# ooowedyn/InkLayer

Hardware: AMD Instinct MI355X
Metric: sketches/sec end-to-end (GroundingDINO+SAM) at 1024x1024 (higher is better)
Workload: dtype f16 (MFMA, f32 accumulate; f32 residual/norm/softmax; split-f16 = fp32-grade operands for patch-embed, neck, mask decoder); 1 GPU; full GroundingDINO Swin-T + SAM ViT-H pipeline, batch=8 per GPU, 1024x1024 synthetic sketches, 16 boxes/sketch, random-init weights; global_batch=8, parallelism=image-parallel x1

## Files before the change

inklayer_amd/csrc/msda.hip:

```cpp
#include "common.h"
#include "../../include/inklayer_hip.h"

namespace {

constexpr int MAXL = 8;

struct LevelInfo {
  int H[MAXL], W[MAXL], start[MAXL];
};

struct HostLevels {
  LevelInfo li;
  __device__ __forceinline__ bool get(int l, int, int& H, int& W, int64_t& start) const {
    H = li.H[l];
    W = li.W[l];
    start = li.start[l];
    return true;
  }
};

struct DevLevels {
  const int64_t* shapes;
  const int64_t* starts;
  __device__ __forceinline__ bool get(int l, int S, int& H, int& W, int64_t& start) const {
    const int64_t h = shapes[2 * l], w = shapes[2 * l + 1], s = starts[l];
    const bool ok = h > 0 && w > 0 && h <= S && w <= S && s >= 0 && s <= S && s + h * w <= S;
    H = ok ? (int)h : 0;
    W = ok ? (int)w : 0;
    start = ok ? s : 0;
    return ok;
  }
};

template <typename T, int NV>
__device__ __forceinline__ void loadv(const T* p, T (&v)[NV]) {
  if constexpr (NV * sizeof(T) % 16 == 0) {
#pragma unroll
    for (int i = 0; i < (int)(NV * sizeof(T) / 16); ++i) {
// ... 21 lines not shown
}

template <typename T, int NV>
__device__ __forceinline__ void sample_acc(const T* __restrict__ vbase, int64_t row_stride, int H, int W,
                                           T h_im, T w_im, T aw, T (&acc)[NV]) {
  if (!(h_im > (T)-1 && w_im > (T)-1 && h_im < (T)H && w_im < (T)W)) return;
  const int h0 = (int)floor(h_im), w0 = (int)floor(w_im);
  const T lh = h_im - (T)h0, lw = w_im - (T)w0;
  const T hh = (T)1 - lh, hw = (T)1 - lw;
  const T w00 = hh * hw * aw, w01 = hh * lw * aw, w10 = lh * hw * aw, w11 = lh * lw * aw;
  T v[NV];
  if (h0 >= 0 && w0 >= 0) {
    loadv<T, NV>(vbase + ((int64_t)h0 * W + w0) * row_stride, v);
#pragma unroll
    for (int i = 0; i < NV; ++i) acc[i] = fma(w00, v[i], acc[i]);
  }
  if (h0 >= 0 && w0 + 1 <= W - 1) {
    loadv<T, NV>(vbase + ((int64_t)h0 * W + w0 + 1) * row_stride, v);
#pragma unroll
    for (int i = 0; i < NV; ++i) acc[i] = fma(w01, v[i], acc[i]);
  }
  if (h0 + 1 <= H - 1 && w0 >= 0) {
    loadv<T, NV>(vbase + ((int64_t)(h0 + 1) * W + w0) * row_stride, v);
#pragma unroll
    for (int i = 0; i < NV; ++i) acc[i] = fma(w10, v[i], acc[i]);
  }
  if (h0 + 1 <= H - 1 && w0 + 1 <= W - 1) {
    loadv<T, NV>(vbase + ((int64_t)(h0 + 1) * W + w0 + 1) * row_stride, v);
#pragma unroll
    for (int i = 0; i < NV; ++i) acc[i] = fma(w11, v[i], acc[i]);
  }
}

__device__ __forceinline__ void sample_acc_bf(const f16* __restrict__ vbase, int64_t row_stride, int H, int W, float h_im,
                                              float w_im, float aw, float (&acc)[8]) {
  const bool in = h_im > -1.f && w_im > -1.f && h_im < (float)H && w_im < (float)W;
  const float hf = floorf(h_im), wf = floorf(w_im);
  const int h0 = in ? (int)hf : 0, w0 = in ? (int)wf : 0;
  const float lh = h_im - hf, lw = w_im - wf;
  const float hh = 1.f - lh, hw = 1.f - lw;
  const bool t = h0 >= 0, b = h0 + 1 <= H - 1, l = w0 >= 0, r = w0 + 1 <= W - 1;
  const float w00 = (in && t && l) ? hh * hw * aw : 0.f, w01 = (in && t && r) ? hh * lw * aw : 0.f;
  const float w10 = (in && b && l) ? lh * hw * aw : 0.f, w11 = (in && b && r) ? lh * lw * aw : 0.f;
  const int ht = max(h0, 0), hb = min(h0 + 1, H - 1), wl = max(w0, 0), wr = min(w0 + 1, W - 1);
  const f16x8 v00 = *(const f16x8*)(vbase + ((int64_t)ht * W + wl) * row_stride);
  const f16x8 v01 = *(const f16x8*)(vbase + ((int64_t)ht * W + wr) * row_stride);
  const f16x8 v10 = *(const f16x8*)(vbase + ((int64_t)hb * W + wl) * row_stride);
  const f16x8 v11 = *(const f16x8*)(vbase + ((int64_t)hb * W + wr) * row_stride);
#pragma unroll
  for (int i = 0; i < 8; ++i) acc[i] = fmaf(w00, (float)v00[i], acc[i]);
#pragma unroll
  for (int i = 0; i < 8; ++i) acc[i] = fmaf(w01, (float)v01[i], acc[i]);
#pragma unroll
  for (int i = 0; i < 8; ++i) acc[i] = fmaf(w10, (float)v10[i], acc[i]);
#pragma unroll
  for (int i = 0; i < 8; ++i) acc[i] = fmaf(w11, (float)v11[i], acc[i]);
}

template <typename T, int NV, typename Levels>
__global__ __launch_bounds__(256) void msda_fwd_kernel(const T* __restrict__ value, const T* __restrict__ loc,
                                                       const T* __restrict__ aw, Levels lv, int B, int S, int M,
                                                       int C, int Q, int L, int P, T* __restrict__ out) {
  const int nsl = C / NV;
  const int gid = xcd_remap(blockIdx.x, gridDim.x) * 256 + threadIdx.x;
  const int qm = gid / nsl, sl = gid - qm * nsl;
  if (qm >= B * Q * M) return;
  const int m = qm % M, b = qm / M / Q;
  T acc[NV];
#pragma unroll
  for (int i = 0; i < NV; ++i) acc[i] = 0;
  const T* lp = loc + (int64_t)qm * L * P * 2;
  const T* wp = aw + (int64_t)qm * L * P;
  const int64_t rs = (int64_t)M * C;
  for (int l = 0; l < L; ++l) {
    int H, W;
    int64_t start;
    if (!lv.get(l, S, H, W, start)) continue;
    const T* vb = value + ((int64_t)b * S + start) * rs + m * C + sl * NV;
    for (int p = 0; p < P; ++p) {
      const T lx = lp[(l * P + p) * 2], ly = lp[(l * P + p) * 2 + 1];
      sample_acc<T, NV>(vb, rs, H, W, ly * (T)H - (T)0.5, lx * (T)W - (T)0.5, wp[l * P + p], acc);
    }
  }
  storev<T, NV>(out + (int64_t)qm * C + sl * NV, acc);
}

template <int G, typename T>
__device__ __forceinline__ T group_sum(T v) {
#pragma unroll
// ... 53 lines not shown
            if (k10) atomicAdd(gval + o10 + c, w10 * ag);
            if (k11) atomicAdd(gval + o11 + c, w11 * ag);
          }
        }
      }
      sa = group_sum<G>(sa);
      sx = group_sum<G>(sx);
      sy = group_sum<G>(sy);
      if (lane == 0) {
        gaw[i] = sa;
        gloc[2 * i] = (T)W * a * sx;
        gloc[2 * i + 1] = (T)H * a * sy;
      }
    }
  }
}

template <int REFD>
__global__ __launch_bounds__(256) void msda_fused_kernel(const f16* __restrict__ value,
                                                         const float* __restrict__ proj, int64_t ldp,
                                                         const float* __restrict__ ref,
                                                         int64_t ref_q_stride, int64_t ref_b_stride,
                                                         LevelInfo li, int B, int S, int Q,
                                                         f16* __restrict__ out) {
  constexpr int M = 8, L = 4, P = 4, C = 32;
  const int64_t gid = (int64_t)xcd_remap(blockIdx.x, gridDim.x) * 256 + threadIdx.x;
  const int c8 = (int)(gid & 3);
  const int64_t qm = gid >> 2;
  if (qm >= (int64_t)B * Q * M) return;
  const int m = (int)(qm % M);
  const int64_t bq = qm / M;
  const int b = (int)(bq / Q), q = (int)(bq % Q);
  const float* pr = proj + bq * ldp;
  float off[L * P * 2], lg[L * P];
#pragma unroll
  for (int i = 0; i < 8; ++i) {
    const f32x4 v = *(const f32x4*)(pr + m * 32 + 4 * i);
    off[4 * i] = v[0]; off[4 * i + 1] = v[1]; off[4 * i + 2] = v[2]; off[4 * i + 3] = v[3];
  }
  float mx = -3.0e38f;
#pragma unroll
  for (int i = 0; i < 4; ++i) {
    const f32x4 v = *(const f32x4*)(pr + 256 + m * 16 + 4 * i);
#pragma unroll
    for (int j = 0; j < 4; ++j) { lg[4 * i + j] = v[j]; mx = fmaxf(mx, v[j]); }
  }
  float sum = 0.f;
#pragma unroll
  for (int i = 0; i < 16; ++i) { lg[i] = expf(lg[i] - mx); sum += lg[i]; }
  const float inv = 1.f / sum;
  const float* rp = ref + (int64_t)b * ref_b_stride + (int64_t)q * ref_q_stride;
  float acc[8] = {0, 0, 0, 0, 0, 0, 0, 0};
  const int64_t rs = (int64_t)M * C;
#pragma unroll
  for (int l = 0; l < L; ++l) {
    const int H = li.H[l], W = li.W[l];
    const f16* vb = value + ((int64_t)b * S + li.start[l]) * rs + m * C + c8 * 8;
    float rx, ry, rw = 0.f, rh = 0.f;
    if (REFD == 2) {
      rx = rp[0]; ry = rp[1];
    } else {
      rx = rp[0]; ry = rp[1]; rw = rp[2]; rh = rp[3];
    }
#pragma unroll
    for (int p = 0; p < P; ++p) {
      const float ox = off[(l * P + p) * 2], oy = off[(l * P + p) * 2 + 1];
      float lx, ly;
      if (REFD == 2) {
        lx = rx + ox / (float)W;
        ly = ry + oy / (float)H;
      } else {
        lx = rx + ox / (float)P * rw * 0.5f;
        ly = ry + oy / (float)P * rh * 0.5f;
      }
      sample_acc_bf(vb, rs, H, W, ly * H - 0.5f, lx * W - 0.5f, lg[l * P + p] * inv, acc);
    }
  }
  f16x8 o;
#pragma unroll
  for (int i = 0; i < 8; ++i) o[i] = (f16)acc[i];
  *(f16x8*)(out + qm * C + c8 * 8) = o;
}

template <typename T, int NV, typename Levels>
int launch_fwd(const void* value, const void* loc, const void* aw, Levels lv, int B, int S, int M, int C, int Q,
               int L, int P, void* out, hipStream_t s) {
  const int64_t threads = (int64_t)B * Q * M * (C / NV);
  hipLaunchKernelGGL((msda_fwd_kernel<T, NV, Levels>), dim3((unsigned)((threads + 255) / 256)), dim3(256), 0, s,
                     (const T*)value, (const T*)loc, (const T*)aw, lv, B, S, M, C, Q, L, P, (T*)out);
  return ink_launch_status();
}

template <typename T, int NVMAX, typename Levels>
int dispatch_fwd(const void* value, const void* loc, const void* aw, Levels lv, int B, int S, int M, int C, int Q,
                 int L, int P, void* out, hipStream_t s) {
  const bool aligned = ink_aligned<16>(value, out);
  if (aligned && C % NVMAX == 0) return launch_fwd<T, NVMAX>(value, loc, aw, lv, B, S, M, C, Q, L, P, out, s);
  if (aligned && C % (NVMAX / 2) == 0) return launch_fwd<T, NVMAX / 2>(value, loc, aw, lv, B, S, M, C, Q, L, P, out, s);
  return launch_fwd<T, 1>(value, loc, aw, lv, B, S, M, C, Q, L, P, out, s);
}

template <typename T, int G, int K>
int launch_bwd(const void* value, DevLevels lv, const void* loc, const void* aw, const void* gout, int B, int S,
               int M, int C, int Q, int L, int P, void* gval, void* gloc, void* gaw, hipStream_t s) {
  const int64_t threads = (int64_t)B * Q * M * G;
  hipLaunchKernelGGL((msda_bwd_kernel<T, G, K>), dim3((unsigned)((threads + 255) / 256)), dim3(256), 0, s,
                     (const T*)value, lv, (const T*)loc, (const T*)aw, (const T*)gout, B, S, M, C, Q, L, P, (T*)gval,
                     (T*)gloc, (T*)gaw);
  return ink_launch_status();
// ... 120 lines not shown
```

inklayer_amd/build.py:

```python
from __future__ import annotations

import os
import subprocess
import sys
from concurrent.futures import ThreadPoolExecutor
from pathlib import Path

ROOT = Path(__file__).resolve().parent
CSRC = ROOT / "csrc"
LIBDIR = ROOT / "lib"
OBJDIR = LIBDIR / "obj"
LIB = LIBDIR / "libinklayer_hip.so"
HIPCC = os.environ.get("HIPCC", "/opt/rocm/bin/hipcc")
FLAGS = ["--offload-arch=gfx950", "-O3", "-std=c++17", "-fPIC", "-ffp-contract=off",
         "-mllvm", "-amdgpu-mfma-vgpr-form",

         "-Wall", "-Wno-unused-function", "-Wno-unused-variable"]


def _newest_header() -> float:
    hs = list(CSRC.glob("*.h")) + list((ROOT.parent / "include").glob("*.h"))
    return max(h.stat().st_mtime for h in hs)


NO_SPILL = {"ffn_fused.hip", "proj_ln.hip", "amg.hip", "layers.hip", "inpaint_ops.hip", "visualize.hip", "evaluate.hip",
            "gemm.hip", "attention_swin.hip", "biattn_wide.hip", "text_bert.hip"}


def _check_no_spill(src: Path, remarks: str) -> None:
    name = None
    for line in remarks.splitlines():
        if "Function Name:" in line:
            name = line.split("Function Name:")[1].split("[")[0].strip()
        elif "ScratchSize [bytes/lane]:" in line:
            n = int(line.split("ScratchSize [bytes/lane]:")[1].split("[")[0])
            if n != 0:
                raise RuntimeError(f"{src.name}: kernel {name} spills ({n} bytes of scratch per lane) - the kernels of "
                                   f"this file must stay in registers (see NO_SPILL); reduce register pressure")


def _compile(src: Path, force: bool, hdr_time: float) -> Path:
    obj = OBJDIR / (src.stem + ".o")
    if (not force and obj.exists() and obj.stat().st_mtime > src.stat().st_mtime
            and obj.stat().st_mtime > hdr_time):
        return obj
    guard = src.name in NO_SPILL
    cmd = [HIPCC, *FLAGS, *(["-Rpass-analysis=kernel-resource-usage", "-fno-caret-diagnostics"] if guard else []), "-c", str(src), "-o", str(obj)]
    r = subprocess.run(cmd, capture_output=True, text=True)
    if r.returncode != 0:
        raise RuntimeError(f"hipcc failed for {src.name}:\n{r.stdout}\n{r.stderr}")
    err = r.stderr
    if guard:
        try:
            _check_no_spill(src, err)
        except RuntimeError:
            obj.unlink(missing_ok=True)
            raise
        err = "\n".join(l for l in err.splitlines()
                        if "kernel-resource-usage" not in l and not l.startswith("In file included from"))
# ... 28 lines not shown
```

inklayer_amd/csrc/attn_few.hip:

```cpp
#include "common.h"
#include "../../include/inklayer_hip.h"

namespace {

__device__ __forceinline__ void load8(const f16* p, float* d) {
  const f16x8 v = *(const f16x8*)p;
#pragma unroll
  for (int j = 0; j < 8; ++j) d[j] = (float)v[j];
}
__device__ __forceinline__ void load8(const float* p, float* d) {
  const f32x4 a = *(const f32x4*)p, b = *(const f32x4*)(p + 4);
#pragma unroll
  for (int j = 0; j < 4; ++j) { d[j] = a[j]; d[4 + j] = b[j]; }
}
__device__ __forceinline__ void store8(f16* p, const float* d) {
  f16x8 v;
#pragma unroll
  for (int j = 0; j < 8; ++j) v[j] = (f16)d[j];
  *(f16x8*)p = v;
}
__device__ __forceinline__ void store8(float* p, const float* d) {
  *(f32x4*)p = (f32x4){d[0], d[1], d[2], d[3]};
  *(f32x4*)(p + 4) = (f32x4){d[4], d[5], d[6], d[7]};
}
// ... 107 lines not shown
      bm = fmaxf(bm, d);
    }
    if (bm <= -1.0e38f) continue;
    const float mn = fmaxf(m, bm);
    const float a = expf(m - mn);
    l *= a;
#pragma unroll
    for (int i = 0; i < HD; ++i) acc[i] *= a;
    m = mn;
#pragma unroll
    for (int u = 0; u < 8; ++u) {
      if (sc[u] <= -1.0e38f) continue;
      const float pw = expf(sc[u] - m);
      l += pw;
      const f16* vp = V + ((int64_t)b * n_k + t0 + u) * ldv + h * HD;
#pragma unroll
      for (int i = 0; i < HD / 8; ++i) {
        float vv[8];
        load8(vp + 8 * i, vv);
#pragma unroll
        for (int j = 0; j < 8; ++j) acc[8 * i + j] = fmaf(pw, vv[j], acc[8 * i + j]);
      }
    }
  }
  const float inv = l > 0.f ? 1.f / l : 0.f;
#pragma unroll
  for (int i = 0; i < HD; ++i) acc[i] *= inv;
  f16* op = O + bq * ldo + h * HD;
#pragma unroll
  for (int i = 0; i < HD / 8; ++i) store8(op + 8 * i, acc + 8 * i);
}


template <int NK>
__global__ __launch_bounds__(256) void attn_fewkeys16_f32_kernel(const float* __restrict__ Q, int64_t ldq,
                                                                 const float* __restrict__ K, int64_t ldk,
                                                                 const float* __restrict__ V, int64_t ldv, int B,
                                                                 int n_q, int n_heads, float scale,
                                                                 const int32_t* __restrict__ q_rows,
                                                                 const float* __restrict__ q_add,
                                                                 float* __restrict__ O, int64_t ldo) {
  const int64_t gid = (int64_t)blockIdx.x * 256 + threadIdx.x;
  if (gid >= (int64_t)B * n_q * n_heads * 4) return;
  const int part = (int)(gid & 3);
  const int h = (int)((gid >> 2) % n_heads);
  const int64_t bq = (gid >> 2) / n_heads;
  const int b = (int)(bq / n_q), q = (int)(bq % n_q);
  const int col = h * 16 + 4 * part;
  f32x4 qv = *(const f32x4*)(Q + (q_rows ? (int64_t)q_rows[b] + q : bq) * ldq + col);
  if (q_add) qv += *(const f32x4*)(q_add + (int64_t)q * n_heads * 16 + col);
  qv *= scale * 1.44269504088896340736f;
  const float* kp = K + (int64_t)b * NK * ldk + col;
  const float* vp = V + (int64_t)b * NK * ldv + col;
  f32x4 kv[NK], vv[NK];
#pragma unroll
  for (int t = 0; t < NK; ++t) {
    kv[t] = *(const f32x4*)(kp + (int64_t)t * ldk);
    vv[t] = *(const f32x4*)(vp + (int64_t)t * ldv);
  }
  float sc[NK];
  float mx = -3.0e38f;
#pragma unroll
  for (int t = 0; t < NK; ++t) {
    float d = (qv[0] * kv[t][0] + qv[1] * kv[t][1]) + (qv[2] * kv[t][2] + qv[3] * kv[t][3]);
    d += __builtin_bit_cast(float, __builtin_amdgcn_update_dpp(0, __builtin_bit_cast(int, d), 0xB1, 0xF, 0xF, false));
    d += __builtin_bit_cast(float, __builtin_amdgcn_update_dpp(0, __builtin_bit_cast(int, d), 0x4E, 0xF, 0xF, false));
    sc[t] = d;
    mx = fmaxf(mx, d);
  }
  float sum = 0.f;
#pragma unroll
  for (int t = 0; t < NK; ++t) { sc[t] = __builtin_amdgcn_exp2f(sc[t] - mx); sum += sc[t]; }
  const float inv = 1.f / sum;
  f32x4 acc = {0.f, 0.f, 0.f, 0.f};
#pragma unroll
  for (int t = 0; t < NK; ++t) acc += (sc[t] * inv) * vv[t];
  *(f32x4*)(O + bq * ldo + col) = acc;
}

template <int QW>
__global__ __launch_bounds__(512) void attn_fewq16_kernel(const float* __restrict__ Q, int64_t ldq,
                                                          const float* __restrict__ K, int64_t ldk,
                                                          const float* __restrict__ V, int64_t ldv, int n_q,
                                                          int n_k, int n_heads, float scale,
                                                          const int32_t* __restrict__ q_rows,
                                                          const int32_t* __restrict__ kv_rows,
                                                          const float* __restrict__ k_add,
                                                          float* __restrict__ O, int64_t ldo) {
  constexpr int KSPLIT = 2, HD = 16, HB = 4, TK = 64;
  constexpr int ROWE = HB * HD;
  constexpr int CH = 4, NCH = ROWE / CH;
  constexpr int NU = TK * NCH / 256;
  constexpr bool Q_IN_LDS = QW > 2;
  extern __shared__ __attribute__((aligned(16))) char fewq_smem[];
  const int grp = threadIdx.x >> 8;
  float* sk = (float*)fewq_smem + grp * 2 * TK * ROWE;
  float* sv = sk + TK * ROWE;
  const int hgroups = n_heads / HB;
  const int b = blockIdx.x / hgroups, h0 = (blockIdx.x % hgroups) * HB;
  const int tid = threadIdx.x & 255, lane = tid & 63, wave = tid >> 6;
  const int per = ((n_k + KSPLIT - 1) / KSPLIT + TK - 1) / TK * TK;
  const int k_lo = grp * per, k_hi = min(n_k, k_lo + per);
  const int kl = lane >> 2, hl = lane & 3;
  const int64_t q0 = q_rows ? (int64_t)q_rows[b] : (int64_t)b * n_q;
  const int64_t k0 = kv_rows ? (int64_t)kv_rows[b] : (int64_t)b * n_k;
  float* sq = (float*)fewq_smem + KSPLIT * 2 * TK * ROWE;
  float qr[QW][HD];
  if (!Q_IN_LDS || (grp == 0 && kl == 0)) {
    const float sc2 = scale * 1.44269504088896340736f;
#pragma unroll
    for (int j = 0; j < QW; ++j) {
      const int qi = QW * wave + j;
      const float* pq = Q + (q0 + (qi < n_q ? qi : 0)) * ldq + (h0 + hl) * HD;
      load8(pq, qr[j]);
      load8(pq + 8, qr[j] + 8);
#pragma unroll
      for (int e = 0; e < HD; ++e) qr[j][e] *= sc2;
      if constexpr (Q_IN_LDS) {
        store8(sq + (qi * HB + hl) * HD, qr[j]);
        store8(sq + (qi * HB + hl) * HD + 8, qr[j] + 8);
      }
    }
  }
  float m[QW], l[QW], acc[QW][HD];
#pragma unroll
  for (int j = 0; j < QW; ++j) {
    m[j] = -3.0e38f;
    l[j] = 0.f;
#pragma unroll
    for (int i = 0; i < HD; ++i) acc[j][i] = 0.f;
  }
  f32x4 rk[NU], rv[NU];
  auto fetch = [&](int t0) {
#pragma unroll
    for (int u = 0; u < NU; ++u) {
      const int c = tid + 256 * u, row = c / NCH, col = c % NCH;
      rk[u] = rv[u] = (f32x4){0.f, 0.f, 0.f, 0.f};
      if (t0 + row < k_hi) {
        rk[u] = *(const f32x4*)(K + (k0 + t0 + row) * ldk + h0 * HD + col * CH);
        rv[u] = *(const f32x4*)(V + (k0 + t0 + row) * ldv + h0 * HD + col * CH);
        if (k_add) rk[u] += *(const f32x4*)(k_add + (int64_t)(t0 + row) * n_heads * HD + h0 * HD + col * CH);
      }
    }
  };
  fetch(k_lo);
  for (int t0 = k_lo; t0 < k_lo + per; t0 += TK) {
    __syncthreads();
#pragma unroll
    for (int u = 0; u < NU; ++u) {
      const int c = tid + 256 * u, row = c / NCH, col = c % NCH;
      *(f32x4*)(sk + row * ROWE + col * CH) = rk[u];
      *(f32x4*)(sv + row * ROWE + col * CH) = rv[u];
    }
    __syncthreads();
    if (t0 + TK < k_hi) fetch(t0 + TK);
    float d[QW][TK / 16];
#pragma unroll
    for (int kk = 0; kk < TK / 16; ++kk) {
      const int key = kk * 16 + kl;
      float kf[HD];
      load8(sk + key * ROWE + hl * HD, kf);
      load8(sk + key * ROWE + hl * HD + 8, kf + 8);
      const bool in = t0 + key < k_hi;
#pragma unroll
      for (int j = 0; j < QW; ++j) {
        float qf[HD];
        if constexpr (Q_IN_LDS) {
          load8(sq + ((QW * wave + j) * HB + hl) * HD, qf);
          load8(sq + ((QW * wave + j) * HB + hl) * HD + 8, qf + 8);
        } else {
#pragma unroll
          for (int e = 0; e < HD; ++e) qf[e] = qr[j][e];
        }
        float a0 = 0.f;
#pragma unroll
        for (int e = 0; e < 8; ++e) {
          a0 = fmaf(qf[e], kf[e], a0);
          a0 = fmaf(qf[8 + e], kf[8 + e], a0);
        }
        d[j][kk] = in ? a0 : -3.0e38f;
      }
    }
    float n[QW];
#pragma unroll
    for (int j = 0; j < QW; ++j) {
// ... 69 lines not shown
        const float inv = 1.f / l[j];
#pragma unroll
        for (int i = 0; i < HD; ++i) acc[j][i] *= inv;
        float* op = O + ((int64_t)b * n_q + qi) * ldo + (h0 + hl) * HD;
        store8(op, acc[j]);
        store8(op + 8, acc[j] + 8);
      }
    }
  }
}

}

extern "C" int ink_attn_fewkeys(const void* Q, int64_t ldq, const void* K, int64_t ldk, const void* V,
                                int64_t ldv, int32_t B, int32_t n_q, int32_t n_k, int32_t n_heads,
                                int32_t head_dim, float scale, const uint8_t* blocked,
                                const int32_t* q_batch_rows, const float* q_add, int32_t io_f32, void* O,
                                int64_t ldo, void* stream) {
  INK_CHECK_ARG(Q && K && V && O && B > 0 && n_q > 0 && n_k > 0 && n_k <= 16 && n_heads > 0);
  INK_CHECK_ARG(ldq % 8 == 0 && ldk % 8 == 0 && ldv % 8 == 0 && ldo % 8 == 0);
  INK_CHECK_ARG(io_f32 == 0 || io_f32 == 1);
  INK_CHECK_ARG(ink_aligned<16>(Q, K, V, O, q_add));
  const int64_t total = (int64_t)B * n_q * n_heads;
  const dim3 grid((unsigned)((total + 255) / 256)), block(256);
  hipStream_t s = (hipStream_t)stream;
#define INK_FEWKEYS(HD, T)                                                                                     \
  hipLaunchKernelGGL((attn_fewkeys_kernel<HD, T>), grid, block, 0, s, (const T*)Q, ldq, (const T*)K, ldk,      \
                     (const T*)V, ldv, B, n_q, n_k, n_heads, scale, blocked, q_batch_rows, q_add, (T*)O, ldo)
  if (head_dim == 32 && !io_f32) INK_FEWKEYS(32, f16);
  else if (head_dim == 64 && !io_f32) INK_FEWKEYS(64, f16);
  else if (!io_f32) return INK_ERR_ARG;
  else if (head_dim == 32) INK_FEWKEYS(32, float);
  else if (head_dim == 16 && !blocked && n_k >= 7) {
    const dim3 g4((unsigned)((total * 4 + 255) / 256));
#define INK_FEWKEYS16(NK)                                                                                        \
  case NK:                                                                                                      \
    hipLaunchKernelGGL(attn_fewkeys16_f32_kernel<NK>, g4, block, 0, s, (const float*)Q, ldq, (const float*)K, ldk, \
                       (const float*)V, ldv, B, n_q, n_heads, scale, q_batch_rows, q_add, (float*)O, ldo);         \
    break
    switch (n_k) {
      INK_FEWKEYS16(7); INK_FEWKEYS16(8); INK_FEWKEYS16(9); INK_FEWKEYS16(10); INK_FEWKEYS16(11);
      INK_FEWKEYS16(12); INK_FEWKEYS16(13); INK_FEWKEYS16(14); INK_FEWKEYS16(15); INK_FEWKEYS16(16);
      default: return INK_ERR_ARG;
    }
#undef INK_FEWKEYS16
  } else if (head_dim == 16) INK_FEWKEYS(16, float);
  else return INK_ERR_ARG;
#undef INK_FEWKEYS
  return ink_launch_status();
}

static int midkeys_launch(const void* Q, int64_t ldq, const void* K, int64_t ldk, const void* V, int64_t ldv,
                          int32_t B, int32_t n_q, int32_t n_k, int32_t n_heads, int32_t head_dim, float scale,
                          const uint8_t* blocked, int64_t blocked_stride, const int32_t* k_len, void* O, int64_t ldo,
                          void* stream) {
  INK_CHECK_ARG(Q && K && V && O && B > 0 && n_q > 0 && n_k > 0 && n_k <= 256 && n_heads > 0);
  INK_CHECK_ARG(head_dim == 32 || head_dim == 64);
  INK_CHECK_ARG(ldq % 8 == 0 && ldk % 8 == 0 && ldv % 8 == 0 && ldo % 8 == 0);
  INK_CHECK_ARG(ink_aligned<16>(Q, K, V, O));
  const int64_t total = (int64_t)B * n_q * n_heads;
  const dim3 grid((unsigned)((total + 255) / 256)), block(256);
#define INK_MIDKEYS(HD)                                                                                            \
  hipLaunchKernelGGL(attn_midkeys_kernel<HD>, grid, block, 0, (hipStream_t)stream, (const f16*)Q, ldq,             \
                     (const f16*)K, ldk, (const f16*)V, ldv, B, n_q, n_k, n_heads, scale, blocked, blocked_stride, \
                     k_len, (f16*)O, ldo)
  if (head_dim == 32) INK_MIDKEYS(32); else INK_MIDKEYS(64);
#undef INK_MIDKEYS
  return ink_launch_status();
}

extern "C" int ink_attn_midkeys(const void* Q, int64_t ldq, const void* K, int64_t ldk, const void* V,
                                int64_t ldv, int32_t B, int32_t n_q, int32_t n_k, int32_t n_heads,
                                int32_t head_dim, float scale, const uint8_t* blocked, void* O, int64_t ldo,
                                void* stream) {
  return midkeys_launch(Q, ldq, K, ldk, V, ldv, B, n_q, n_k, n_heads, head_dim, scale, blocked, 0, nullptr, O, ldo,
                        stream);
}

// ... 28 lines not shown
```

inklayer_amd/csrc/sam_decoder.hip:

```cpp
#include "common.h"
#include "sam_postprocess.h"
#include "../../include/inklayer_hip.h"

namespace {

__device__ __forceinline__ void pe_feature(float x, float y, const float* __restrict__ G, int F, int f, float& sv,
                                           float& cv) {
  const float cx = 2.f * x - 1.f, cy = 2.f * y - 1.f;
  float v = cx * G[f] + cy * G[F + f];
  v = 6.283185307179586f * v;
  sv = sinf(v);
  cv = cosf(v);
}

__global__ __launch_bounds__(256) void pe_encode_kernel(const float* __restrict__ coords,
                                                        const float* __restrict__ G, int N, int F,
                                                        const float* __restrict__ add, int n_add,
                                                        float* __restrict__ out) {
  const int i = blockIdx.x * 256 + threadIdx.x;
  if (i >= N * F) return;
  const int n = i / F, f = i % F;
  float sv, cv;
  pe_feature(coords[2 * n], coords[2 * n + 1], G, F, f, sv, cv);
  if (add) {
// ... 166 lines not shown
  const int b = (int)(tok / ((int64_t)g * g));
  const float* u = up + r * C;
  const float* h = hyper + (int64_t)b * C;
  float acc = 0.f;
#pragma unroll
  for (int c = 0; c < C; c += 4) {
    const f32x4 uv = *(const f32x4*)(u + c);
    const f32x4 hv = *(const f32x4*)(h + c);
    acc = fmaf(hv[0], uv[0], acc);
    acc = fmaf(hv[1], uv[1], acc);
    acc = fmaf(hv[2], uv[2], acc);
    acc = fmaf(hv[3], uv[3], acc);
  }
  const int Y = 4 * y + 2 * (s1 >> 1) + (s2 >> 1), X = 4 * x + 2 * (s1 & 1) + (s2 & 1);
  out[((int64_t)b * 4 * g + Y) * 4 * g + X] = acc;
}

__global__ __launch_bounds__(256) void postprocess_kernel(const float* __restrict__ low, int n, int S,
                                                          int L, int in_h, int in_w, int out_h,
                                                          int out_w, float thr,
                                                          uint8_t* __restrict__ out,
                                                          float* __restrict__ out_logits) {
  const int64_t total = (int64_t)n * out_h * out_w;
  const PostScales sc = post_scales(S, L, in_h, in_w, out_h, out_w);
  for (int64_t i = (int64_t)blockIdx.x * 256 + threadIdx.x; i < total; i += (int64_t)gridDim.x * 256) {
    const int X = (int)(i % out_w), Y = (int)((i / out_w) % out_h);
    const int b = (int)(i / ((int64_t)out_w * out_h));
    const float v = post_pixel(low + (int64_t)b * S * S, S, sc, in_h, in_w, Y, X);
    if (out) out[i] = v > thr ? 1 : 0;
    if (out_logits) out_logits[i] = v;
  }
}

__global__ __launch_bounds__(256) void postprocess_rows_kernel(const float* __restrict__ low, int n, int S, int L,
                                                               int in_h, int in_w, int out_h, int out_w, float thr,
                                                               uint8_t* __restrict__ out,
                                                               float* __restrict__ out_logits) {
  constexpr int PX = 4;
  const float sA = (float)S / (float)L;
  const float sBh = (float)in_h / (float)out_h, sBw = (float)in_w / (float)out_w;
  const int wq = out_w / PX;
  for (int xq = threadIdx.x; xq < wq; xq += 256) {
    float lx[PX], lc[PX][2];
    int c0[PX][2], c1[PX][2];
#pragma unroll
    for (int px = 0; px < PX; ++px) {
      int x0, x1;
      bil(xq * PX + px, sBw, in_w, x0, x1, lx[px]);
      bil(x0, sA, S, c0[px][0], c1[px][0], lc[px][0]);
      bil(x1, sA, S, c0[px][1], c1[px][1], lc[px][1]);
    }
    for (int row = blockIdx.x; row < n * out_h; row += gridDim.x) {
      const int b = row / out_h, Y = row - b * out_h;
      const float* lp = low + (int64_t)b * S * S;
      int y0, y1;
      float ly;
      bil(Y, sBh, in_h, y0, y1, ly);
      int a0[2], a1[2];
      float la[2];
      bil(y0, sA, S, a0[0], a1[0], la[0]);
      bil(y1, sA, S, a0[1], a1[1], la[1]);
      const float* r00 = lp + a0[0] * S;
      const float* r01 = lp + a1[0] * S;
      const float* r10 = lp + a0[1] * S;
      const float* r11 = lp + a1[1] * S;
      float vals[PX];
#pragma unroll
      for (int px = 0; px < PX; ++px) {
        auto stageA = [&](const float* ra, const float* rb, float lav, int k) {
          const float v00 = ra[c0[px][k]], v01 = ra[c1[px][k]];
          const float v10 = rb[c0[px][k]], v11 = rb[c1[px][k]];
          return (1.f - lav) * ((1.f - lc[px][k]) * v00 + lc[px][k] * v01) + lav * ((1.f - lc[px][k]) * v10 + lc[px][k] * v11);
        };
        const float v00 = stageA(r00, r01, la[0], 0), v01 = stageA(r00, r01, la[0], 1);
        const float v10 = stageA(r10, r11, la[1], 0), v11 = stageA(r10, r11, la[1], 1);
        vals[px] = (1.f - ly) * ((1.f - lx[px]) * v00 + lx[px] * v01) + ly * ((1.f - lx[px]) * v10 + lx[px] * v11);
      }
      const int64_t o = (int64_t)row * out_w + (int64_t)xq * PX;
      if (out)
        *(uint32_t*)(out + o) = (uint32_t)(vals[0] > thr) | ((uint32_t)(vals[1] > thr) << 8) |
                                ((uint32_t)(vals[2] > thr) << 16) | ((uint32_t)(vals[3] > thr) << 24);
      if (out_logits) *(f32x4*)(out_logits + o) = (f32x4){vals[0], vals[1], vals[2], vals[3]};
    }
  }
}

}

extern "C" int ink_sam_pe_encode(const float* coords01, const float* gauss, int32_t N, int32_t F,
                                 const float* add, int32_t n_add, float* out, void* stream) {
  INK_CHECK_ARG(coords01 && gauss && out && N > 0 && F > 0 && (!add || n_add > 0));
  hipLaunchKernelGGL(pe_encode_kernel, dim3((N * F + 255) / 256), dim3(256), 0, (hipStream_t)stream,
                     coords01, gauss, N, F, add, n_add, out);
  return ink_launch_status();
}

extern "C" int ink_sam_mask_logits(const float* up, const float* hyper, int32_t n, int32_t g,
                                   int32_t C, float* out, void* stream) {
  INK_CHECK_ARG(up && hyper && out && n > 0 && g > 0);
  const int64_t total = (int64_t)n * g * g * 16;
  const dim3 grid((unsigned)((total + 255) / 256)), block(256);
  if (C == 32) {
    hipLaunchKernelGGL(mask_logits_kernel<32>, grid, block, 0, (hipStream_t)stream, up, hyper, n, g, out);
  } else if (C == 8) {
    hipLaunchKernelGGL(mask_logits_kernel<8>, grid, block, 0, (hipStream_t)stream, up, hyper, n, g, out);
  } else {
    return INK_ERR_ARG;
  }
  return ink_launch_status();
}

extern "C" int ink_sam_postprocess(const float* low, int32_t n, int32_t S, int32_t L, int32_t in_h,
                                   int32_t in_w, int32_t out_h, int32_t out_w, float thr,
                                   void* out_u8, float* out_logits, void* stream) {
  INK_CHECK_ARG(low && (out_u8 || out_logits) && n > 0 && S > 0 && L >= S);
  INK_CHECK_ARG(in_h > 0 && in_w > 0 && in_h <= L && in_w <= L && out_h > 0 && out_w > 0);
  const int64_t total = (int64_t)n * out_h * out_w;
  if (out_w % 4 == 0 && (int64_t)n * out_h < (int64_t)1 << 30 && ink_aligned<4>(out_u8) &&
      ink_aligned<16>(out_logits)) {
    const int64_t rows = (int64_t)n * out_h;
    const int blocks = (int)(rows < 8192 ? rows : 8192);
    hipLaunchKernelGGL(postprocess_rows_kernel, dim3(blocks), dim3(256), 0, (hipStream_t)stream, low, n, S, L, in_h,
                       in_w, out_h, out_w, thr, (uint8_t*)out_u8, out_logits);
    return ink_launch_status();
  }
  const int blocks = (int)((total + 255) / 256 < 16384 ? (total + 255) / 256 : 16384);
  hipLaunchKernelGGL(postprocess_kernel, dim3(blocks), dim3(256), 0, (hipStream_t)stream, low, n, S,
                     L, in_h, in_w, out_h, out_w, thr, (uint8_t*)out_u8, out_logits);
  return ink_launch_status();
}

extern "C" int ink_sam_prompt_tokens(const float* points, const int32_t* labels, int32_t n_pts, int32_t pad,
                                     const float* boxes, const float* gauss, int32_t F, const float* point_emb,
                                     const float* not_a_point, const float* out_tok, float input_size, int32_t P,
                                     float* out, void* stream) {
  INK_CHECK_ARG(gauss && point_emb && not_a_point && out_tok && out && P > 0 && F > 0 && input_size > 0.f);
  INK_CHECK_ARG(n_pts >= 0 && (n_pts == 0 || (points && labels)) && (pad == 0 || pad == 1));
  const int NT = 5 + n_pts + pad + (boxes ? 2 : 0);
  INK_CHECK_ARG(NT <= 16);
  const int64_t total = (int64_t)P * NT * F;
  hipLaunchKernelGGL(prompt_tokens_kernel, dim3((unsigned)((total + 255) / 256)), dim3(256), 0, (hipStream_t)stream,
                     points, labels, n_pts, pad, boxes, gauss, F, point_emb, not_a_point, out_tok, input_size, P, NT, out);
  return ink_launch_status();
}

extern "C" int ink_sam_mask_embed(const float* mask, const float* emb, const int32_t* emb_rows, const float* params,
                                  int32_t n_params, float eps, int32_t P, int32_t g, float* keys, void* split_f16,
                                  void* stream) {
  INK_CHECK_ARG(mask && emb && emb_rows && params && keys && P > 0 && g > 0 && g <= 64 && n_params == MP_TOTAL);
  INK_CHECK_ARG(ink_aligned<16>(mask, emb, keys) && ink_aligned<8>(split_f16));
  hipLaunchKernelGGL(mask_embed_kernel, dim3((unsigned)(P * g)), dim3(256), 0, (hipStream_t)stream, mask, emb, emb_rows,
                     params, eps, g, keys, (f16*)split_f16);
  return ink_launch_status();
}
```

Baseline: 119.3 sketches/s.

## Share MSDA sampling geometry across quad lanes with DPP broadcasts and mixed FMA

In the fused deformable-attention kernel, each of the four lanes serving one (query, head) now computes the bilinear geometry and softmax logit for just one sampling point per level, not all 16 points. Weights and row indices are broadcast within the quad with DPP. Softmax max and sum are reduced across the quad the same way. Value loads use 32-bit offsets and v_fma_mix_f32, so f16 values feed f32 accumulators without separate conversions. This cuts the redundant per-lane geometry, exp and offset-load work, in exchange for cross-lane DPP traffic, inline asm, and the risk of 32-bit byte-offset overflow on large value tensors.

```diff
diff --git a/inklayer_amd/csrc/msda.hip b/inklayer_amd/csrc/msda.hip
--- a/inklayer_amd/csrc/msda.hip
+++ b/inklayer_amd/csrc/msda.hip
@@ -4,6 +4,8 @@
 namespace {
 
 constexpr int MAXL = 8;
+
+typedef uint32_t u32x4 __attribute__((ext_vector_type(4)));
 
 struct LevelInfo {
   int H[MAXL], W[MAXL], start[MAXL];
@@ -91,29 +93,61 @@
   }
 }
 
-__device__ __forceinline__ void sample_acc_bf(const f16* __restrict__ vbase, int64_t row_stride, int H, int W, float h_im,
-                                              float w_im, float aw, float (&acc)[8]) {
+__device__ __forceinline__ void sample_geom(int H, int W, int start, float h_im, float w_im, float aw, float (&w)[4],
+                                            int (&row)[4]) {
   const bool in = h_im > -1.f && w_im > -1.f && h_im < (float)H && w_im < (float)W;
   const float hf = floorf(h_im), wf = floorf(w_im);
   const int h0 = in ? (int)hf : 0, w0 = in ? (int)wf : 0;
   const float lh = h_im - hf, lw = w_im - wf;
   const float hh = 1.f - lh, hw = 1.f - lw;
   const bool t = h0 >= 0, b = h0 + 1 <= H - 1, l = w0 >= 0, r = w0 + 1 <= W - 1;
-  const float w00 = (in && t && l) ? hh * hw * aw : 0.f, w01 = (in && t && r) ? hh * lw * aw : 0.f;
-  const float w10 = (in && b && l) ? lh * hw * aw : 0.f, w11 = (in && b && r) ? lh * lw * aw : 0.f;
+  w[0] = (in && t && l) ? hh * hw * aw : 0.f;
+  w[1] = (in && t && r) ? hh * lw * aw : 0.f;
+  w[2] = (in && b && l) ? lh * hw * aw : 0.f;
+  w[3] = (in && b && r) ? lh * lw * aw : 0.f;
   const int ht = max(h0, 0), hb = min(h0 + 1, H - 1), wl = max(w0, 0), wr = min(w0 + 1, W - 1);
-  const f16x8 v00 = *(const f16x8*)(vbase + ((int64_t)ht * W + wl) * row_stride);
-  const f16x8 v01 = *(const f16x8*)(vbase + ((int64_t)ht * W + wr) * row_stride);
-  const f16x8 v10 = *(const f16x8*)(vbase + ((int64_t)hb * W + wl) * row_stride);
-  const f16x8 v11 = *(const f16x8*)(vbase + ((int64_t)hb * W + wr) * row_stride);
-#pragma unroll
-  for (int i = 0; i < 8; ++i) acc[i] = fmaf(w00, (float)v00[i], acc[i]);
-#pragma unroll
-  for (int i = 0; i < 8; ++i) acc[i] = fmaf(w01, (float)v01[i], acc[i]);
-#pragma unroll
-  for (int i = 0; i < 8; ++i) acc[i] = fmaf(w10, (float)v10[i], acc[i]);
-#pragma unroll
-  for (int i = 0; i < 8; ++i) acc[i] = fmaf(w11, (float)v11[i], acc[i]);
+  row[0] = start + ht * W + wl;
+  row[1] = start + ht * W + wr;
+  row[2] = start + hb * W + wl;
+  row[3] = start + hb * W + wr;
+}
+
+template <int SRC>
+__device__ __forceinline__ int quad_bcast(int x) {
+  return __builtin_amdgcn_update_dpp(0, x, SRC * 0x55, 0xF, 0xF, true);
+}
+template <int SRC>
+__device__ __forceinline__ float quad_bcast(float x) {
+  return __builtin_bit_cast(float, quad_bcast<SRC>(__builtin_bit_cast(int, x)));
+}
+
+template <int HI>
+__device__ __forceinline__ void fma_f16_half(float w, uint32_t pair, float& acc) {
+  if constexpr (HI)
+    asm("v_fma_mix_f32 %0, %1, %2, %0 op_sel:[0,1,0] op_sel_hi:[0,1,0]" : "+v"(acc) : "v"(w), "v"(pair));
+  else
+    asm("v_fma_mix_f32 %0, %1, %2, %0 op_sel:[0,0,0] op_sel_hi:[0,1,0]" : "+v"(acc) : "v"(w), "v"(pair));
+}
+
+template <int SRC>
+__device__ __forceinline__ void quad_sample_acc(const char* __restrict__ vbase, uint32_t row_bytes, const float (&w)[4],
+                                                const int (&row)[4], float (&acc)[8]) {
+  float wb[4];
+  u32x4 v[4];
+#pragma unroll
+  for (int k = 0; k < 4; ++k) {
+    wb[k] = quad_bcast<SRC>(w[k]);
+    const uint32_t r = (uint32_t)quad_bcast<SRC>(row[k]);
+    v[k] = *(const u32x4*)(vbase + (uint64_t)r * row_bytes);
+  }
+#pragma unroll
+  for (int k = 0; k < 4; ++k) {
+#pragma unroll
+    for (int i = 0; i < 4; ++i) {
+      fma_f16_half<0>(wb[k], v[k][i], acc[2 * i]);
+      fma_f16_half<1>(wb[k], v[k][i], acc[2 * i + 1]);
+    }
+  }
 }
 
 template <typename T, int NV, typename Levels>
@@ -233,49 +267,57 @@
   const int64_t bq = qm / M;
   const int b = (int)(bq / Q), q = (int)(bq % Q);
   const float* pr = proj + bq * ldp;
-  float off[L * P * 2], lg[L * P];
-#pragma unroll
-  for (int i = 0; i < 8; ++i) {
-    const f32x4 v = *(const f32x4*)(pr + m * 32 + 4 * i);
-    off[4 * i] = v[0]; off[4 * i + 1] = v[1]; off[4 * i + 2] = v[2]; off[4 * i + 3] = v[3];
-  }
+  float ox[L], oy[L], e[L];
   float mx = -3.0e38f;
 #pragma unroll
-  for (int i = 0; i < 4; ++i) {
-    const f32x4 v = *(const f32x4*)(pr + 256 + m * 16 + 4 * i);
-#pragma unroll
-    for (int j = 0; j < 4; ++j) { lg[4 * i + j] = v[j]; mx = fmaxf(mx, v[j]); }
-  }
+  for (int l = 0; l < L; ++l) {
+    const f32x2 o = *(const f32x2*)(pr + m * 32 + (l * P + c8) * 2);
+    ox[l] = o[0];
+    oy[l] = o[1];
+    e[l] = pr[256 + m * 16 + l * P + c8];
+    mx = fmaxf(mx, e[l]);
+  }
+  mx = fmaxf(mx, __builtin_bit_cast(float, __builtin_amdgcn_update_dpp(0, __builtin_bit_cast(int, mx), 0xB1, 0xF, 0xF, true)));
+  mx = fmaxf(mx, __builtin_bit_cast(float, __builtin_amdgcn_update_dpp(0, __builtin_bit_cast(int, mx), 0x4E, 0xF, 0xF, true)));
   float sum = 0.f;
 #pragma unroll
-  for (int i = 0; i < 16; ++i) { lg[i] = expf(lg[i] - mx); sum += lg[i]; }
+  for (int l = 0; l < L; ++l) {
+    e[l] = expf(e[l] - mx);
+    sum += quad_bcast<0>(e[l]);
+    sum += quad_bcast<1>(e[l]);
+    sum += quad_bcast<2>(e[l]);
+    sum += quad_bcast<3>(e[l]);
+  }
   const float inv = 1.f / sum;
   const float* rp = ref + (int64_t)b * ref_b_stride + (int64_t)q * ref_q_stride;
+  float rx, ry, rw = 0.f, rh = 0.f;
+  if (REFD == 2) {
+    rx = rp[0]; ry = rp[1];
+  } else {
+    rx = rp[0]; ry = rp[1]; rw = rp[2]; rh = rp[3];
+  }
   float acc[8] = {0, 0, 0, 0, 0, 0, 0, 0};
-  const int64_t rs = (int64_t)M * C;
+  const char* vb = (const char*)(value + (int64_t)b * S * (M * C) + m * C + c8 * 8);
+  uint32_t row_bytes = M * C * sizeof(f16);
+  asm("" : "+s"(row_bytes));
 #pragma unroll
   for (int l = 0; l < L; ++l) {
     const int H = li.H[l], W = li.W[l];
-    const f16* vb = value + ((int64_t)b * S + li.start[l]) * rs + m * C + c8 * 8;
-    float rx, ry, rw = 0.f, rh = 0.f;
+    float lx, ly;
     if (REFD == 2) {
-      rx = rp[0]; ry = rp[1];
+      lx = rx + ox[l] / (float)W;
+      ly = ry + oy[l] / (float)H;
     } else {
-      rx = rp[0]; ry = rp[1]; rw = rp[2]; rh = rp[3];
-    }
-#pragma unroll
-    for (int p = 0; p < P; ++p) {
-      const float ox = off[(l * P + p) * 2], oy = off[(l * P + p) * 2 + 1];
-      float lx, ly;
-      if (REFD == 2) {
-        lx = rx + ox / (float)W;
-        ly = ry + oy / (float)H;
-      } else {
-        lx = rx + ox / (float)P * rw * 0.5f;
-        ly = ry + oy / (float)P * rh * 0.5f;
-      }
-      sample_acc_bf(vb, rs, H, W, ly * H - 0.5f, lx * W - 0.5f, lg[l * P + p] * inv, acc);
-    }
+      lx = rx + ox[l] / (float)P * rw * 0.5f;
+      ly = ry + oy[l] / (float)P * rh * 0.5f;
+    }
+    float w[4];
+    int row[4];
+    sample_geom(H, W, li.start[l], ly * H - 0.5f, lx * W - 0.5f, e[l] * inv, w, row);
+    quad_sample_acc<0>(vb, row_bytes, w, row, acc);
+    quad_sample_acc<1>(vb, row_bytes, w, row, acc);
+    quad_sample_acc<2>(vb, row_bytes, w, row, acc);
+    quad_sample_acc<3>(vb, row_bytes, w, row, acc);
   }
   f16x8 o;
 #pragma unroll
```

Measured after the change: 119.8 sketches/s (median of 6 runs). Within noise of the previous version (+0.4%).

## Stage postprocess source rows in LDS and batch fewkeys16 attention per block

Applied to the files above, without the earlier changes.

The SAM postprocess kernel now processes 16-row chunks. It stages the needed low-res source rows into shared memory once per chunk and precomputes per-row interpolation indices. An identity-resize variant skips the second bilinear stage and falls back to an exact per-pixel path for zero or non-finite values. The few-keys head_dim-16 attention kernel now handles several query rows per thread so K/V loads are reused, and the few-query kernel defers the k_add addition to the shared-memory store. Together these add complexity, extra syncs and new fallback paths, and both files join the no-spill guard.

```diff
diff --git a/inklayer_amd/build.py b/inklayer_amd/build.py
--- a/inklayer_amd/build.py
+++ b/inklayer_amd/build.py
@@ -24,7 +24,7 @@
 
 
 NO_SPILL = {"ffn_fused.hip", "proj_ln.hip", "amg.hip", "layers.hip", "inpaint_ops.hip", "visualize.hip", "evaluate.hip",
-            "gemm.hip", "attention_swin.hip", "biattn_wide.hip", "text_bert.hip"}
+            "gemm.hip", "attention_swin.hip", "biattn_wide.hip", "text_bert.hip", "attn_few.hip", "sam_decoder.hip"}
 
 
 def _check_no_spill(src: Path, remarks: str) -> None:
diff --git a/inklayer_amd/csrc/attn_few.hip b/inklayer_amd/csrc/attn_few.hip
--- a/inklayer_amd/csrc/attn_few.hip
+++ b/inklayer_amd/csrc/attn_few.hip
@@ -163,7 +163,8 @@
 }
 
 
-template <int NK>
+constexpr int FEWKEYS16_U = 4;
+template <int NK, int U>
 __global__ __launch_bounds__(256) void attn_fewkeys16_f32_kernel(const float* __restrict__ Q, int64_t ldq,
                                                                  const float* __restrict__ K, int64_t ldk,
                                                                  const float* __restrict__ V, int64_t ldv, int B,
@@ -171,16 +172,24 @@
                                                                  const int32_t* __restrict__ q_rows,
                                                                  const float* __restrict__ q_add,
                                                                  float* __restrict__ O, int64_t ldo) {
-  const int64_t gid = (int64_t)blockIdx.x * 256 + threadIdx.x;
-  if (gid >= (int64_t)B * n_q * n_heads * 4) return;
-  const int part = (int)(gid & 3);
-  const int h = (int)((gid >> 2) % n_heads);
-  const int64_t bq = (gid >> 2) / n_heads;
-  const int b = (int)(bq / n_q), q = (int)(bq % n_q);
-  const int col = h * 16 + 4 * part;
-  f32x4 qv = *(const f32x4*)(Q + (q_rows ? (int64_t)q_rows[b] + q : bq) * ldq + col);
-  if (q_add) qv += *(const f32x4*)(q_add + (int64_t)q * n_heads * 16 + col);
-  qv *= scale * 1.44269504088896340736f;
+  const int LR = n_heads * 4;
+  const int64_t per = (int64_t)n_q * LR;
+  const int nb = (int)((per + 256 * U - 1) / (256 * U));
+  const int b = blockIdx.x / nb;
+  const int64_t f0 = (int64_t)(blockIdx.x - b * nb) * (256 * U) + threadIdx.x;
+  const int col = (int)(f0 % LR) * 4;
+  const int64_t qrow0 = q_rows ? (int64_t)q_rows[b] : (int64_t)b * n_q;
+  f32x4 qv[U];
+#pragma unroll
+  for (int u = 0; u < U; ++u) {
+    const int64_t f = f0 + 256 * u;
+    qv[u] = (f32x4){0.f, 0.f, 0.f, 0.f};
+    if (f < per) {
+      const int q = (int)(f / LR);
+      qv[u] = *(const f32x4*)(Q + (qrow0 + q) * ldq + col);
+      if (q_add) qv[u] += *(const f32x4*)(q_add + (int64_t)q * n_heads * 16 + col);
+    }
+  }
   const float* kp = K + (int64_t)b * NK * ldk + col;
   const float* vp = V + (int64_t)b * NK * ldv + col;
   f32x4 kv[NK], vv[NK];
@@ -189,24 +198,30 @@
     kv[t] = *(const f32x4*)(kp + (int64_t)t * ldk);
     vv[t] = *(const f32x4*)(vp + (int64_t)t * ldv);
   }
-  float sc[NK];
-  float mx = -3.0e38f;
-#pragma unroll
-  for (int t = 0; t < NK; ++t) {
-    float d = (qv[0] * kv[t][0] + qv[1] * kv[t][1]) + (qv[2] * kv[t][2] + qv[3] * kv[t][3]);
-    d += __builtin_bit_cast(float, __builtin_amdgcn_update_dpp(0, __builtin_bit_cast(int, d), 0xB1, 0xF, 0xF, false));
-    d += __builtin_bit_cast(float, __builtin_amdgcn_update_dpp(0, __builtin_bit_cast(int, d), 0x4E, 0xF, 0xF, false));
-    sc[t] = d;
-    mx = fmaxf(mx, d);
-  }
-  float sum = 0.f;
-#pragma unroll
-  for (int t = 0; t < NK; ++t) { sc[t] = __builtin_amdgcn_exp2f(sc[t] - mx); sum += sc[t]; }
-  const float inv = 1.f / sum;
-  f32x4 acc = {0.f, 0.f, 0.f, 0.f};
-#pragma unroll
-  for (int t = 0; t < NK; ++t) acc += (sc[t] * inv) * vv[t];
-  *(f32x4*)(O + bq * ldo + col) = acc;
+#pragma unroll
+  for (int u = 0; u < U; ++u) {
+    const int64_t f = f0 + 256 * u;
+    if (f >= per) break;
+    const f32x4 qs = qv[u] * (scale * 1.44269504088896340736f);
+    float sc[NK];
+    float mx = -3.0e38f;
+#pragma unroll
+    for (int t = 0; t < NK; ++t) {
+      float d = (qs[0] * kv[t][0] + qs[1] * kv[t][1]) + (qs[2] * kv[t][2] + qs[3] * kv[t][3]);
+      d += __builtin_bit_cast(float, __builtin_amdgcn_update_dpp(0, __builtin_bit_cast(int, d), 0xB1, 0xF, 0xF, false));
+      d += __builtin_bit_cast(float, __builtin_amdgcn_update_dpp(0, __builtin_bit_cast(int, d), 0x4E, 0xF, 0xF, false));
+      sc[t] = d;
+      mx = fmaxf(mx, d);
+    }
+    float sum = 0.f;
+#pragma unroll
+    for (int t = 0; t < NK; ++t) { sc[t] = __builtin_amdgcn_exp2f(sc[t] - mx); sum += sc[t]; }
+    const float inv = 1.f / sum;
+    f32x4 acc = {0.f, 0.f, 0.f, 0.f};
+#pragma unroll
+    for (int t = 0; t < NK; ++t) acc += (sc[t] * inv) * vv[t];
+    *(f32x4*)(O + ((int64_t)b * n_q + (int)(f / LR)) * ldo + col) = acc;
+  }
 }
 
 template <int QW>
@@ -261,16 +276,24 @@
 #pragma unroll
     for (int i = 0; i < HD; ++i) acc[j][i] = 0.f;
   }
-  f32x4 rk[NU], rv[NU];
+  constexpr bool ADD_AT_STORE = QW == 2;
+  struct Stage {
+    f32x4 k[NU], v[NU], a[ADD_AT_STORE ? NU : 1];
+  };
+  Stage r;
   auto fetch = [&](int t0) {
 #pragma unroll
     for (int u = 0; u < NU; ++u) {
       const int c = tid + 256 * u, row = c / NCH, col = c % NCH;
-      rk[u] = rv[u] = (f32x4){0.f, 0.f, 0.f, 0.f};
+      r.k[u] = r.v[u] = (f32x4){0.f, 0.f, 0.f, 0.f};
       if (t0 + row < k_hi) {
-        rk[u] = *(const f32x4*)(K + (k0 + t0 + row) * ldk + h0 * HD + col * CH);
-        rv[u] = *(const f32x4*)(V + (k0 + t0 + row) * ldv + h0 * HD + col * CH);
-        if (k_add) rk[u] += *(const f32x4*)(k_add + (int64_t)(t0 + row) * n_heads * HD + h0 * HD + col * CH);
+        r.k[u] = *(const f32x4*)(K + (k0 + t0 + row) * ldk + h0 * HD + col * CH);
+        r.v[u] = *(const f32x4*)(V + (k0 + t0 + row) * ldv + h0 * HD + col * CH);
+        if (k_add) {
+          const f32x4 ka = *(const f32x4*)(k_add + (int64_t)(t0 + row) * n_heads * HD + h0 * HD + col * CH);
+          if constexpr (ADD_AT_STORE) r.a[u] = ka;
+          else r.k[u] += ka;
+        }
       }
     }
   };
@@ -280,8 +303,11 @@
 #pragma unroll
     for (int u = 0; u < NU; ++u) {
       const int c = tid + 256 * u, row = c / NCH, col = c % NCH;
-      *(f32x4*)(sk + row * ROWE + col * CH) = rk[u];
-      *(f32x4*)(sv + row * ROWE + col * CH) = rv[u];
+      if constexpr (ADD_AT_STORE) {
+        if (k_add && t0 + row < k_hi) r.k[u] += r.a[u];
+      }
+      *(f32x4*)(sk + row * ROWE + col * CH) = r.k[u];
+      *(f32x4*)(sv + row * ROWE + col * CH) = r.v[u];
     }
     __syncthreads();
     if (t0 + TK < k_hi) fetch(t0 + TK);
@@ -417,11 +443,17 @@
   else if (!io_f32) return INK_ERR_ARG;
   else if (head_dim == 32) INK_FEWKEYS(32, float);
   else if (head_dim == 16 && !blocked && n_k >= 7) {
-    const dim3 g4((unsigned)((total * 4 + 255) / 256));
-#define INK_FEWKEYS16(NK)                                                                                        \
-  case NK:                                                                                                      \
-    hipLaunchKernelGGL(attn_fewkeys16_f32_kernel<NK>, g4, block, 0, s, (const float*)Q, ldq, (const float*)K, ldk, \
-                       (const float*)V, ldv, B, n_q, n_heads, scale, q_batch_rows, q_add, (float*)O, ldo);         \
+    const bool multi = 256 % (n_heads * 4) == 0;
+    const int64_t per = (int64_t)n_q * n_heads * 4, span = multi ? 256 * FEWKEYS16_U : 256;
+    const int64_t nblk = (int64_t)B * ((per + span - 1) / span);
+    INK_CHECK_ARG(nblk < (int64_t)1 << 31);
+    const dim3 g4((unsigned)nblk);
+#define INK_FEWKEYS16_U(NK, U)                                                                                   \
+  hipLaunchKernelGGL((attn_fewkeys16_f32_kernel<NK, U>), g4, block, 0, s, (const float*)Q, ldq, (const float*)K, \
+                     ldk, (const float*)V, ldv, B, n_q, n_heads, scale, q_batch_rows, q_add, (float*)O, ldo)
+#define INK_FEWKEYS16(NK)                                                     \
+  case NK:                                                                    \
+    if (multi) INK_FEWKEYS16_U(NK, FEWKEYS16_U); else INK_FEWKEYS16_U(NK, 1); \
     break
     switch (n_k) {
       INK_FEWKEYS16(7); INK_FEWKEYS16(8); INK_FEWKEYS16(9); INK_FEWKEYS16(10); INK_FEWKEYS16(11);
@@ -429,6 +461,7 @@
       default: return INK_ERR_ARG;
     }
 #undef INK_FEWKEYS16
+#undef INK_FEWKEYS16_U
   } else if (head_dim == 16) INK_FEWKEYS(16, float);
   else return INK_ERR_ARG;
 #undef INK_FEWKEYS
diff --git a/inklayer_amd/csrc/sam_decoder.hip b/inklayer_amd/csrc/sam_decoder.hip
--- a/inklayer_amd/csrc/sam_decoder.hip
+++ b/inklayer_amd/csrc/sam_decoder.hip
@@ -222,15 +222,28 @@
   }
 }
 
+constexpr int POST_ROWS = 16;
+constexpr int POST_TILE = 6144;
+template <bool IDENT>
 __global__ __launch_bounds__(256) void postprocess_rows_kernel(const float* __restrict__ low, int n, int S, int L,
                                                                int in_h, int in_w, int out_h, int out_w, float thr,
                                                                uint8_t* __restrict__ out,
-                                                               float* __restrict__ out_logits) {
+                                                               float* __restrict__ out_logits, int tx_log2) {
   constexpr int PX = 4;
+  typedef int i32x4 __attribute__((ext_vector_type(4)));
+  __shared__ float tile[POST_TILE];
+  __shared__ i32x4 row_at[POST_ROWS];
+  __shared__ f32x4 row_w[POST_ROWS];
   const float sA = (float)S / (float)L;
   const float sBh = (float)in_h / (float)out_h, sBw = (float)in_w / (float)out_w;
+  const PostScales sc{sA, sBh, sBw};
   const int wq = out_w / PX;
-  for (int xq = threadIdx.x; xq < wq; xq += 256) {
+  const int TX = 1 << tx_log2, TY = 256 >> tx_log2;
+  const int tx = threadIdx.x & (TX - 1), ty = threadIdx.x >> tx_log2;
+  const int chunks_per = (out_h + POST_ROWS - 1) / POST_ROWS;
+  const int chunks = n * chunks_per;
+  for (int xb = 0; xb < wq; xb += TX) {
+    const int xq = xb + tx;
     float lx[PX], lc[PX][2];
     int c0[PX][2], c1[PX][2];
 #pragma unroll
@@ -240,37 +253,87 @@
       bil(x0, sA, S, c0[px][0], c1[px][0], lc[px][0]);
       bil(x1, sA, S, c0[px][1], c1[px][1], lc[px][1]);
     }
-    for (int row = blockIdx.x; row < n * out_h; row += gridDim.x) {
-      const int b = row / out_h, Y = row - b * out_h;
+    for (int chunk = blockIdx.x; chunk < chunks; chunk += gridDim.x) {
+      const int b = chunk / chunks_per, Y0 = (chunk - b * chunks_per) * POST_ROWS;
+      const int Y1 = min(Y0 + POST_ROWS, out_h) - 1;
       const float* lp = low + (int64_t)b * S * S;
-      int y0, y1;
-      float ly;
-      bil(Y, sBh, in_h, y0, y1, ly);
-      int a0[2], a1[2];
-      float la[2];
-      bil(y0, sA, S, a0[0], a1[0], la[0]);
-      bil(y1, sA, S, a0[1], a1[1], la[1]);
-      const float* r00 = lp + a0[0] * S;
-      const float* r01 = lp + a1[0] * S;
-      const float* r10 = lp + a0[1] * S;
-      const float* r11 = lp + a1[1] * S;
-      float vals[PX];
-#pragma unroll
-      for (int px = 0; px < PX; ++px) {
-        auto stageA = [&](const float* ra, const float* rb, float lav, int k) {
-          const float v00 = ra[c0[px][k]], v01 = ra[c1[px][k]];
-          const float v10 = rb[c0[px][k]], v11 = rb[c1[px][k]];
-          return (1.f - lav) * ((1.f - lc[px][k]) * v00 + lc[px][k] * v01) + lav * ((1.f - lc[px][k]) * v10 + lc[px][k] * v11);
-        };
-        const float v00 = stageA(r00, r01, la[0], 0), v01 = stageA(r00, r01, la[0], 1);
-        const float v10 = stageA(r10, r11, la[1], 0), v11 = stageA(r10, r11, la[1], 1);
-        vals[px] = (1.f - ly) * ((1.f - lx[px]) * v00 + lx[px] * v01) + ly * ((1.f - lx[px]) * v10 + lx[px] * v11);
+      int lo, hi;
+      {
+        int y0, y1, t;
+        float w;
+        bil(Y0, sBh, in_h, y0, y1, w);
+        bil(y0, sA, S, lo, t, w);
+        bil(Y1, sBh, in_h, y0, y1, w);
+        bil(y1, sA, S, t, hi, w);
       }
-      const int64_t o = (int64_t)row * out_w + (int64_t)xq * PX;
-      if (out)
-        *(uint32_t*)(out + o) = (uint32_t)(vals[0] > thr) | ((uint32_t)(vals[1] > thr) << 8) |
-                                ((uint32_t)(vals[2] > thr) << 16) | ((uint32_t)(vals[3] > thr) << 24);
-      if (out_logits) *(f32x4*)(out_logits + o) = (f32x4){vals[0], vals[1], vals[2], vals[3]};
+      const int64_t cnt = (int64_t)(hi - lo + 1) * S;
+      const bool over = cnt > POST_TILE;
+      __syncthreads();
+      bool bad = over;
+      if (!over) {
+        if (threadIdx.x <= Y1 - Y0) {
+          int y0, y1, a0[2], a1[2];
+          float ly, la[2];
+          bil(Y0 + threadIdx.x, sBh, in_h, y0, y1, ly);
+          bil(y0, sA, S, a0[0], a1[0], la[0]);
+          bil(y1, sA, S, a0[1], a1[1], la[1]);
+          row_at[threadIdx.x] = (i32x4){(a0[0] - lo) * S, (a1[0] - lo) * S, (a0[1] - lo) * S, (a1[1] - lo) * S};
+          row_w[threadIdx.x] = (f32x4){la[0], la[1], ly, 0.f};
+        }
+        const float* src = lp + (int64_t)lo * S;
+        for (int i = threadIdx.x; i < (int)cnt; i += 256) {
+          const float v = src[i];
+          tile[i] = v;
+          bad |= !(fabsf(v) <= 1.0e37f);
+        }
+      }
+      const bool slow = IDENT ? (bool)__syncthreads_or(bad) : (__syncthreads(), over);
+      if (xq >= wq) continue;
+      for (int Y = Y0 + ty; Y <= Y1; Y += TY) {
+        const int row = b * out_h + Y;
+        float vals[PX] = {0.f, 0.f, 0.f, 0.f};
+        if (!over) {
+          const i32x4 at = row_at[Y - Y0];
+          const f32x4 rw = row_w[Y - Y0];
+          const float la[2] = {rw[0], rw[1]}, ly = rw[2];
+          const float* r00 = tile + at[0];
+          const float* r01 = tile + at[1];
+          const float* r10 = tile + at[2];
+          const float* r11 = tile + at[3];
+#pragma unroll
+          for (int px = 0; px < PX; ++px) {
+            auto stageA = [&](const float* ra, const float* rb, float lav, int k) {
+              const float v00 = ra[c0[px][k]], v01 = ra[c1[px][k]];
+              const float v10 = rb[c0[px][k]], v11 = rb[c1[px][k]];
+              return (1.f - lav) * ((1.f - lc[px][k]) * v00 + lc[px][k] * v01) + lav * ((1.f - lc[px][k]) * v10 + lc[px][k] * v11);
+            };
+            if constexpr (IDENT) {
+              vals[px] = stageA(r00, r01, la[0], 0);
+            } else {
+              const float v00 = stageA(r00, r01, la[0], 0), v01 = stageA(r00, r01, la[0], 1);
+              const float v10 = stageA(r10, r11, la[1], 0), v11 = stageA(r10, r11, la[1], 1);
+              vals[px] = (1.f - ly) * ((1.f - lx[px]) * v00 + lx[px] * v01) + ly * ((1.f - lx[px]) * v10 + lx[px] * v11);
+            }
+          }
+        }
+        if (slow || (IDENT && (vals[0] == 0.f || vals[1] == 0.f || vals[2] == 0.f || vals[3] == 0.f))) {
+#pragma unroll 1
+          for (int px = 0; px < PX; ++px) {
+            const float cur = px == 0 ? vals[0] : px == 1 ? vals[1] : px == 2 ? vals[2] : vals[3];
+            if (!slow && cur != 0.f) continue;
+            const float v = post_pixel(lp, S, sc, in_h, in_w, Y, xq * PX + px);
+            vals[0] = px == 0 ? v : vals[0];
+            vals[1] = px == 1 ? v : vals[1];
+            vals[2] = px == 2 ? v : vals[2];
+            vals[3] = px == 3 ? v : vals[3];
+          }
+        }
+        const int64_t o = (int64_t)row * out_w + (int64_t)xq * PX;
+        if (out)
+          *(uint32_t*)(out + o) = (uint32_t)(vals[0] > thr) | ((uint32_t)(vals[1] > thr) << 8) |
+                                  ((uint32_t)(vals[2] > thr) << 16) | ((uint32_t)(vals[3] > thr) << 24);
+        if (out_logits) *(f32x4*)(out_logits + o) = (f32x4){vals[0], vals[1], vals[2], vals[3]};
+      }
     }
   }
 }
@@ -308,10 +371,13 @@
   const int64_t total = (int64_t)n * out_h * out_w;
   if (out_w % 4 == 0 && (int64_t)n * out_h < (int64_t)1 << 30 && ink_aligned<4>(out_u8) &&
       ink_aligned<16>(out_logits)) {
-    const int64_t rows = (int64_t)n * out_h;
-    const int blocks = (int)(rows < 8192 ? rows : 8192);
-    hipLaunchKernelGGL(postprocess_rows_kernel, dim3(blocks), dim3(256), 0, (hipStream_t)stream, low, n, S, L, in_h,
-                       in_w, out_h, out_w, thr, (uint8_t*)out_u8, out_logits);
+    const int chunks = n * ((out_h + POST_ROWS - 1) / POST_ROWS);
+    int tx_log2 = 0;
+    while (tx_log2 < 8 && (1 << tx_log2) < out_w / 4) ++tx_log2;
+    const bool ident = in_h == out_h && in_w == out_w && in_h < (1 << 23) && in_w < (1 << 23);
+    hipLaunchKernelGGL(ident ? postprocess_rows_kernel<true> : postprocess_rows_kernel<false>, dim3(chunks), dim3(256),
+                       0, (hipStream_t)stream, low, n, S, L, in_h, in_w, out_h, out_w, thr, (uint8_t*)out_u8,
+                       out_logits, tx_log2);
     return ink_launch_status();
   }
   const int blocks = (int)((total + 255) / 256 < 16384 ? (total + 255) / 256 : 16384);
```

Result: no change. 119.2 sketches/s before, 120.0 sketches/s after (median of 4 runs) (+0.7%).
